# wzx99/DCFP

Hardware: AMD Instinct MI355X
Metric: training images/sec at 1024x2048 DeepLabv3-R101 (higher is better)
Workload: dtype f32; 1 GPU; DeepLabv3-resnet101+ASPP os8, 4x3x1024x2048 per GPU, CE+0.4*deepsup CE (fused upsample), 3x3 stride-1 convs with >= 256 channels as fp32 Winograd F(2x2,3x3) (fwd / dgrad / wgrad), all other convs direct implicit GEMM, EIC step, SGD m0.9 wd5e-4; global_batch=4, parallelism=dp1

## Files before the change

dcfp_amd/_lib.py:

```python
import ctypes as C
import os
import subprocess
import threading

_HERE = os.path.dirname(os.path.abspath(__file__))
LIB_PATH = os.environ.get("DCFP_LIB") or os.path.join(_HERE, "libdcfp_hip.so")
CSRC = os.path.join(_HERE, "csrc")

_lib = None
_lock = threading.Lock()


class ConvDesc(C.Structure):
    _fields_ = [(n, C.c_int32) for n in
                ("N", "Cin", "H", "W", "Cout", "KH", "KW", "stride", "pad", "dil", "Hout", "Wout",
                 "x_pitch", "dy_pitch")]


class ConvF16Desc(C.Structure):
    _fields_ = [(n, C.c_int32) for n in
                ("N", "H", "W", "Cin8", "x_pitch", "Cout", "K", "stride", "pad", "dil", "Hout", "Wout",
                 "y_pitch", "y_off", "res_pitch", "res_off", "relu")]


# ... 86 lines not shown
    "dcfp_p2p_import": (_I, [_P, C.POINTER(C.c_void_p)]),
    "dcfp_p2p_unmap": (_I, [_P]),
    "dcfp_syncbn_p2p_exchange_f32": (_I, [C.POINTER(C.c_void_p), _I, _I, C.c_uint32, _I, _P, _I, _I, _P, _R,
                                          C.c_uint32, _P, _P]),
    "dcfp_bn_apply_relu_mask_f32": (_I, [_P, _P, _P, _P, _P, _F, _P, _P, _P, _I, _I, _I, _P]),
    "dcfp_conv2d_fwd_stat_slots": (_L, [_D, _P, _L]),
    "dcfp_conv2d_fwd_stats_f32_nchw": (_I, [_D, _P, _P, _P, _L, _P, _P, _Z, _I, _P]),
    "dcfp_bn_stats_from_partials_f32": (_I, [_P, _L, _I, _I, _P, _P, _R, _P]),
    "dcfp_bn_bwd_apply_f32": (_I, [_P, _L, _P, _P, _L, _P, _P, _P, _P, _F, _P, _P, _F, _P, _I, _P, _P,
                                   _I, _I, _I, _I, _I, _P]),
    "dcfp_bn_bwd_fused_sync_bytes": (_Z, [_I, _I, _I]),
    "dcfp_bn_bwd_fused_f32": (_I, [_P, _L, _P, _P, _L, _P, _P, _P, _P, _F, _F, _I, _P, _P, _I, _I, _I, _I, _I,
                                   _P, _P, _P, _P, _P, _Z, C.c_uint32, C.c_uint32, _P, _P]),
    "dcfp_maxpool3x3s2_fwd_f32": (_I, [_P, _P, _P, _I, _I, _I, _I, _I, _I, _P]),
    "dcfp_maxpool3x3s2_bwd_f32": (_I, [_P, _P, _P, _I, _I, _I, _I, _I, _I, _P]),
    "dcfp_rowsum_f32": (_I, [_P, _L, _P, _F, _I, _I, _I, _P]),
    "dcfp_broadcast_hw_f32": (_I, [_P, _F, _P, _L, _I, _I, _I, _I, _P]),
    "dcfp_add_f32": (_I, [_P, _P, _P, _L, _P]),
    "dcfp_channel_scale_f32": (_I, [_P, _P, _P, _I, _I, _I, _P]),
    "dcfp_upsample_bilinear_fwd_f32": (_I, [_P, _P, _I, _I, _I, _I, _I, _I, _I, _P]),
    "dcfp_upsample_bilinear_bwd_f32": (_I, [_P, _P, _I, _I, _I, _I, _I, _I, _I, _P]),
    "dcfp_resize_bilinear_into_f32": (_I, [_P, _L, _I, _I, _I, _I, _P, _L, _I, _I, _I, _I, _P]),
    "dcfp_resize_bilinear_adjoint_f32": (_I, [_P, _L, _I, _I, _I, _I, _I, _P, _L, _I, _I, _I, _I, _P]),
    "dcfp_ppm_pool_f32": (_I, [_P, _I, _I, _I, _I, _I, _P, _P, _I, _P, _L, _I, _P]),
    "dcfp_ppm_pool_adjoint_f32": (_I, [_P, _I, _I, _I, _I, _I, _P, _P, _L, _I, _P, _P]),
    "dcfp_ppm_resize_adjoint_f32": (_I, [_P, _L, _I, _I, _I, _I, _I, _P, _P, _I, _P]),
    "dcfp_upsample_ce_workspace_bytes": (_Z, [_I, _I, _I]),
    "dcfp_upsample_ce_fwd_f32": (_I, [_P, _P, _P, _I, _I, _I, _I, _I, _I, _I, _I, _P, _P, _P, _P,
                                      _Z, _P]),
    "dcfp_upsample_ce_bwd_f32": (_I, [_P, _P, _P, _I, _I, _I, _I, _I, _I, _I, _I, _P, _P, _P, _P]),
# ... 74 lines not shown
```

dcfp_amd/csrc/bn.hip:

```cpp
#include "common.h"
#include <stdlib.h>

namespace {

constexpr int kThreads = 256;

__device__ __forceinline__ float bn_val(float v, float mu, float istd, float g, float b) {
    return fmaf((v - mu) * istd, g, b);
}

struct BnPlan {
    int chunks;
    int chunk_elems;
};

constexpr int kChunkElems = 8192;

BnPlan bn_plan(int N, int C, int HW) {
    const long long E = (long long)N * HW;
    long long chunks = (E + kChunkElems - 1) / kChunkElems;
    if (E <= kChunkElems) {
        const long long by_size = (E + 2047) / 2048;
        long long by_grid = 4096 / (C > 0 ? C : 1);
        if (by_grid < 1) by_grid = 1;
// ... 951 lines not shown
```

dcfp_amd/csrc/common.h:

```cpp
#pragma once
#include <hip/hip_runtime.h>
#include <stdint.h>
#include <stddef.h>
#include "../../include/dcfp_hip.h"

#define DCFP_WAVE 64

#define DCFP_RETURN_LAUNCH()                         \
    do {                                             \
        hipError_t e__ = hipGetLastError();          \
        return (e__ == hipSuccess) ? DCFP_OK : (int)e__; \
    } while (0)

struct Igemm2Red {
    const float* x;
    const unsigned long long* mask;
    const float* mean;
    float* part;
};

static inline hipStream_t dcfp_s(dcfp_stream_t s) { return reinterpret_cast<hipStream_t>(s); }

static inline bool dcfp_aligned16(const void* p) { return (reinterpret_cast<uintptr_t>(p) & 15u) == 0; }

// ... 12 lines not shown
    for (int off = 32; off > 0; off >>= 1) v += __shfl_down(v, off, 64);
    return v;
}

__device__ __forceinline__ float block_sum_256(float v, float* smem ) {
    v = wave_sum(v);
    const int lane = threadIdx.x & 63, wid = threadIdx.x >> 6;
    if (lane == 0) smem[wid] = v;
    __syncthreads();
    float r = 0.f;
    if (threadIdx.x == 0) r = (smem[0] + smem[1]) + (smem[2] + smem[3]);
    __syncthreads();
    return r;
}

__device__ __forceinline__ void running_update(const DcfpBnRunning& r, int c, float mean, float var, float n) {
    if (r.running_mean) {
#pragma clang fp contract(off)
        const float unb = n / fmaxf(n - 1.0f, 1.0f);
        const float keep = 1.0f - r.momentum;
        const float a = r.running_mean[c] * keep, b = r.momentum * mean;
        r.running_mean[c] = a + b;
        const float vu = var * unb;
        const float d = r.running_var[c] * keep, e = r.momentum * vu;
        r.running_var[c] = d + e;
    }
    if (c == 0 && r.num_batches_tracked) r.num_batches_tracked[0] += 1;
}
```

dcfp_amd/csrc/conv_igemm2.hip:

```cpp
#include "igemm2_common.h"
#include <queue>
#include <vector>
#include <stdio.h>
#include <stdlib.h>

namespace {

__device__ __forceinline__ int wp_row(int m, int perm8) {
    if (!perm8) return m;
    const int j = m & 255;
    return (m & ~255) + 32 * (j & 7) + (j >> 3);
}

__global__ void __launch_bounds__(256)
permute_weights_kernel(const float* __restrict__ w, float* __restrict__ wp, int T, int Ck, int CkP,
                       int M, int Mpad, int sAm, int sAc, int perm8) {
    const long long total = (long long)T * CkP * Mpad;
    for (long long i = (long long)blockIdx.x * 256 + threadIdx.x; i < total;
         i += (long long)gridDim.x * 256) {
        const int m = wp_row((int)(i % Mpad), perm8);
        const long long r = i / Mpad;
        const int c = (int)(r % CkP);
        const int t = (int)(r / CkP);
        float v = 0.f;
// ... 24 lines not shown
        return;
    }
    const long long total = (long long)e.T * e.CkP * e.Mpad;
#pragma unroll
    for (int u = 0; u < kWpBlockElems / 256; ++u) {
        const long long i = base + u * 256 + threadIdx.x;
        if (i >= total) return;
        const int m = wp_row((int)(i % e.Mpad), e.perm8);
        const long long r = i / e.Mpad;
        const int c = (int)(r % e.CkP);
        const int t = (int)(r / e.CkP);
        float v = 0.f;
        if (m < e.M && c < e.Ck) v = e.w[(long long)m * e.sAm + (long long)c * e.sAc + t];
        e.wp[i] = v;
    }
}

__device__ __forceinline__ float half_xor(float v, int mask) {
    switch (mask) {
        case 1: return __builtin_bit_cast(float, __builtin_amdgcn_ds_swizzle(__builtin_bit_cast(int, v), (1 << 10) | 0x1f));
        case 2: return __builtin_bit_cast(float, __builtin_amdgcn_ds_swizzle(__builtin_bit_cast(int, v), (2 << 10) | 0x1f));
        case 4: return __builtin_bit_cast(float, __builtin_amdgcn_ds_swizzle(__builtin_bit_cast(int, v), (4 << 10) | 0x1f));
        case 8: return __builtin_bit_cast(float, __builtin_amdgcn_ds_swizzle(__builtin_bit_cast(int, v), (8 << 10) | 0x1f));
        default: return __builtin_bit_cast(float, __builtin_amdgcn_ds_swizzle(__builtin_bit_cast(int, v), (16 << 10) | 0x1f));
    }
}

template <int TAPS, int TM, int TN, int WM, int WN, bool SD, bool ACC, int KB = 16>
__global__ void __launch_bounds__(64 * WM * WN, (TM * TN <= 8 && WM * WN == 4 && !ACC) ? 2 : 1)
igemm2_kernel(const Igemm2Params p) {
// ... 915 lines not shown
    if (pick_tapskip(p, 256) == 0) return 1.0;
    long long live = 0;
    for (int ti = 0; ti < p.tiles_per_img; ++ti) live += tile_live_rows(p, ti);
    return (double)live / (3.0 * p.tiles_per_img);
}

void dcfp_igemm2_wp_layout(int T, int M, int Ck, int P, long long px, int sn, int sd, int off0, int offstep, int HiWi,
                           int Wo, bool pitched, int sAm, int sAc, DcfpWpEntry* e) {
    const TileCfg c = pick_cfg(M, px, sd);
    const bool d8 = dcfp_igemm2_use_dma8(T, M, P, px, sn, sd, off0, offstep, HiWi, Wo, pitched);
    e->T = T; e->Ck = Ck; e->CkP = round_up(Ck, ck_pad()); e->M = M; e->Mpad = round_up(M, d8 ? 256 : c.bm);
    e->sAm = sAm; e->sAc = sAc; e->perm8 = d8 ? 1 : 0;
}

int dcfp_igemm2_permute_multi(const DcfpWpEntry* table, int n, long long total_blocks, hipStream_t stream) {
    hipLaunchKernelGGL(permute_weights_multi_kernel, dim3((unsigned)total_blocks), dim3(256), 0, stream, table, n);
    DCFP_RETURN_LAUNCH();
}

bool dcfp_igemm2_persist() {
    static const bool persist = [] { const char* e = getenv("DCFP_IGEMM_PERSIST"); return !e || atoi(e) != 0; }();
    return persist;
}

bool dcfp_igemm2_dma_shape(int T, int M, int Ck, int P, long long px, int sn, int sd, int off0, int HiWi, int Wo) {
    static const bool dma = [] { const char* e = getenv("DCFP_IGEMM_DMA"); return !e || atoi(e) != 0; }();
    static const bool dma9 = [] { const char* e = getenv("DCFP_IGEMM_DMA9"); return !e || atoi(e) != 0; }();
    if (!dma || pick_cfg(M, px, sd).id != 4 || sn != 1 || sd != 1 || HiWi != P || Wo % 4 != 0) return false;
    return T == 1 ? off0 == 0 : dma9;
}

// ... 106 lines not shown
```

dcfp_amd/csrc/igemm2_common.h:

```cpp
#pragma once
#include "common.h"
#include <type_traits>

struct Igemm2Params {
    const float* in;
    const float* wp;
    const float* bias;
    const float* scale;
    const float* shift;
    const float* residual;
    int relu;
    float* out;
    long long in_nstride, out_nstride;
    int N, M, Mpad, Ck, CkP;
    int Hi, Wi, Ho, Wo, P, tiles_per_img, tiles_n_total, tiles_m;
    int sn, sd, off0, offstep;
    int accumulate, vec_store;
    int tile2d;
    int Hc, Wc, tiles_per_phase;
    int in_pitch;
    int zfold;
    const float* fan_src;
    const unsigned long long* fan_mask;
    long long wp_nstride;
// ... 10 lines not shown

typedef float f32x16 __attribute__((ext_vector_type(16)));
typedef float f32x4 __attribute__((ext_vector_type(4)));

constexpr int BK = 16;
constexpr unsigned kOob = 0x80000000u;

template <int I, int N, typename F>
__device__ __forceinline__ void static_for(F&& f) {
    if constexpr (I < N) {
        f(std::integral_constant<int, I>{});
        static_for<I + 1, N>(f);
    }
}

__device__ __forceinline__ void wino_filter2_pair(const float* __restrict__ w, int sAm, int sAc, int flip, int M, int Ck,
                                                  int Mpad, long long idx, float* __restrict__ Ug) {
    const int mblocks = Mpad / 64;
    const int c = (int)(idx / Mpad), m = (int)(idx - (long long)c * Mpad);
    float g[9];
    if (m < M && c < Ck) {
        const float* src = w + (long long)m * sAm + (long long)c * sAc;
#pragma unroll
        for (int t = 0; t < 9; ++t) g[t] = src[flip ? 8 - t : t];
    } else {
#pragma unroll
        for (int t = 0; t < 9; ++t) g[t] = 0.f;
    }
    float r[4][3];
#pragma unroll
    for (int k = 0; k < 3; ++k) {
        const float g0 = g[k], g1 = g[3 + k], g2 = g[6 + k];
        r[0][k] = g0;
        r[1][k] = 0.5f * ((g0 + g2) + g1);
        r[2][k] = 0.5f * ((g0 + g2) - g1);
        r[3][k] = g2;
    }
    const int cb = c >> 3, cl = c & 7, mb = m >> 6, ml = m & 63;
    float* dst = Ug + ((((long long)(cb * mblocks + mb) * 16) * 2 + (ml >> 5)) * 64 + (cl & 1) * 32 + (ml & 31)) * 4 + (cl >> 1);
#pragma unroll
    for (int i = 0; i < 4; ++i) {
        const float a = r[i][0], b = r[i][1], cc = r[i][2];
        dst[(4 * i + 0) * 512] = a;
        dst[(4 * i + 1) * 512] = 0.5f * ((a + cc) + b);
        dst[(4 * i + 2) * 512] = 0.5f * ((a + cc) - b);
        dst[(4 * i + 3) * 512] = cc;
    }
}

template <int T>
struct Frag;
template <>
struct Frag<4> {
    static __device__ __forceinline__ void ld(const float* p, float (&f)[4]) {
        const float4 v = *reinterpret_cast<const float4*>(p);
        f[0] = v.x; f[1] = v.y; f[2] = v.z; f[3] = v.w;
    }
};
template <>
struct Frag<2> {
    static __device__ __forceinline__ void ld(const float* p, float (&f)[2]) {
        const float2 v = *reinterpret_cast<const float2*>(p);
// ... 10 lines not shown
```

dcfp_amd/csrc/pool.hip:

```cpp
#include "common.h"
#include <math.h>

namespace {

constexpr int kThreads = 256;

__global__ void __launch_bounds__(kThreads)
maxpool3x3s2_fwd_kernel(const float* __restrict__ x, float* __restrict__ y,
                        int32_t* __restrict__ argmax, long long total, int H, int W, int Hout,
                        int Wout) {
    for (long long idx = (long long)blockIdx.x * kThreads + threadIdx.x; idx < total;
         idx += (long long)gridDim.x * kThreads) {
        const int ow = (int)(idx % Wout);
        const long long t = idx / Wout;
        const int oh = (int)(t % Hout);
        const long long plane = t / Hout;
        const float* xp = x + plane * (long long)H * W;
        const int h0 = oh * 2 - 1, w0 = ow * 2 - 1;
        const int hs = h0 < 0 ? 0 : h0, ws = w0 < 0 ? 0 : w0;
        const int he = h0 + 3 > H ? H : h0 + 3, we = w0 + 3 > W ? W : w0 + 3;
        float best = -INFINITY;
        int bi = hs * W + ws;
        for (int h = hs; h < he; ++h) {
            for (int w = ws; w < we; ++w) {
// ... 21 lines not shown
    const float* xp = x + plane * (long long)H * W;
    const int h0 = 2 * oh - 1, c0 = 2 * ow0;
    float best[4] = {-INFINITY, -INFINITY, -INFINITY, -INFINITY};
    const int hs = h0 < 0 ? 0 : h0;
    int bi[4];
#pragma unroll
    for (int j = 0; j < 4; ++j) bi[j] = hs * W + ((c0 + 2 * j - 1) < 0 ? 0 : (c0 + 2 * j - 1));
#pragma unroll
    for (int r = 0; r < 3; ++r) {
        const int h = h0 + r;
        if (h < 0 || h >= H) continue;
        const float* row = xp + (long long)h * W;
        const float4 a = *reinterpret_cast<const float4*>(row + c0);
        const float4 b = *reinterpret_cast<const float4*>(row + c0 + 4);
        const float v[9] = {c0 > 0 ? row[c0 - 1] : 0.f, a.x, a.y, a.z, a.w, b.x, b.y, b.z, b.w};
#pragma unroll
        for (int j = 0; j < 4; ++j) {
#pragma unroll
            for (int k = 0; k < 3; ++k) {
                if (k == 0 && j == 0 && c0 == 0) continue;
                const float t = v[2 * j + k];
                if (t > best[j] || t != t) { best[j] = t; bi[j] = h * W + c0 + 2 * j + k - 1; }
            }
        }
    }
    const long long o = rowid * Wout + ow0;
    *reinterpret_cast<float4*>(y + o) = make_float4(best[0], best[1], best[2], best[3]);
    *reinterpret_cast<int4*>(argmax + o) = make_int4(bi[0], bi[1], bi[2], bi[3]);
}

// ... 161 lines not shown
    if (Hout != (H + 2 - 3) / 2 + 1 || Wout != (W + 2 - 3) / 2 + 1) return DCFP_E_BADDESC;
    if ((long long)H * W > 0x7fffffffLL) return DCFP_E_UNSUPPORTED;
    const long long total = (long long)N * C * Hout * Wout;
    const long long orows = (long long)N * C * Hout;
    const int segs = (Wout / 4 + kThreads - 1) / kThreads;
    if (W % 8 == 0 && dcfp_aligned16(x) && dcfp_aligned16(y) && dcfp_aligned16(argmax) &&
        orows * segs <= 0x7fffffffLL)
        hipLaunchKernelGGL(maxpool3x3s2_fwd_vec4_kernel, dim3((unsigned)(orows * segs)), dim3(kThreads), 0,
                           dcfp_s(stream), x, y, argmax, H, W, Hout, Wout, segs);
    else
        hipLaunchKernelGGL(maxpool3x3s2_fwd_kernel, dim3(stream_grid(total)), dim3(kThreads), 0,
                           dcfp_s(stream), x, y, argmax, total, H, W, Hout, Wout);
    DCFP_RETURN_LAUNCH();
}

extern "C" int dcfp_maxpool3x3s2_bwd_f32(const float* dy, const int32_t* argmax, float* dx, int N,
                                         int C, int H, int W, int Hout, int Wout,
                                         dcfp_stream_t stream) {
    if (!dy || !dx || !argmax || N <= 0 || C <= 0 || H <= 0 || W <= 0) return DCFP_E_BADDESC;
    if (Hout != (H + 2 - 3) / 2 + 1 || Wout != (W + 2 - 3) / 2 + 1) return DCFP_E_BADDESC;
    const long long total = (long long)N * C * H * W;
    const long long rows = (long long)N * C * H;
    const int segs = (W / 4 + kThreads - 1) / kThreads;
    if (W % 4 == 0 && dcfp_aligned16(dx) && rows * segs <= 0x7fffffffLL)
        hipLaunchKernelGGL(maxpool3x3s2_bwd_vec4_kernel, dim3((unsigned)(rows * segs)), dim3(kThreads), 0,
                           dcfp_s(stream), dy, argmax, dx, H, W, Hout, Wout, segs);
    else
        hipLaunchKernelGGL(maxpool3x3s2_bwd_kernel, dim3(stream_grid(total)), dim3(kThreads), 0,
                           dcfp_s(stream), dy, argmax, dx, total, H, W, Hout, Wout);
    DCFP_RETURN_LAUNCH();
// ... 44 lines not shown
```

dcfp_amd/networks/_exec.py:

```python
import os

import torch
import torch.nn as nn

from .. import ops

_BN_TYPES = (nn.BatchNorm2d, nn.SyncBatchNorm)


def conv(m, x):
    if m.groups != 1 or m.kernel_size[0] != m.kernel_size[1] or m.stride[0] != m.stride[1] \
            or m.padding[0] != m.padding[1] or m.dilation[0] != m.dilation[1] \
            or isinstance(m.padding, str) or m.padding_mode != "zeros":
        raise RuntimeError(f"dcfp_amd: unsupported conv configuration {m}")
    return ops.conv2d(x, m.weight, m.bias, m.stride[0], m.padding[0], m.dilation[0])


FUSE_BLOCKS = os.environ.get("DCFP_NO_BLOCK_FUSION") is None


def _bn_args(m):
    training = m.training or (m.running_mean is None)
    sync = False
    if isinstance(m, nn.SyncBatchNorm) and training:
# ... 43 lines not shown
            shift = bn.bias - bn.running_mean * scale
        cached = (key, scale.contiguous(), shift.contiguous())
        bn._dcfp_fold = cached
    return cached[1], cached[2]


def conv_bn_act(cm, bn, x, relu=False, residual=None, next_conv=None):
    if (not bn.training) and bn.running_mean is not None and not torch.is_grad_enabled() \
            and cm.bias is None and cm.groups == 1 and cm.padding_mode == "zeros":
        scale, shift = _fold(bn)
        return ops.conv2d_fused_infer(x, cm.weight, scale, shift, cm.stride[0], cm.padding[0],
                                      cm.dilation[0], residual, relu)
    return bn_act(bn, conv(cm, x), relu=relu, residual=residual, prev_conv=cm, next_conv=next_conv)


def _plain_conv(m, k):
    ok = (m.groups == 1 and m.bias is None and m.kernel_size == (k, k) and m.padding_mode == "zeros"
          and not isinstance(m.padding, str))
    if not ok:
        raise RuntimeError(f"dcfp_amd: unsupported conv configuration in Bottleneck: {m}")


def bottleneck(blk, x):
    _plain_conv(blk.conv1, 1); _plain_conv(blk.conv2, 3); _plain_conv(blk.conv3, 1)
    bns = [blk.bn1, blk.bn2, blk.bn3]
    tensors = [blk.conv1.weight, blk.bn1.weight, blk.bn1.bias, blk.conv2.weight, blk.bn2.weight,
               blk.bn2.bias, blk.conv3.weight, blk.bn3.weight, blk.bn3.bias]
    stride, dil = blk.conv2.stride[0], blk.conv2.dilation[0]
    if blk.conv2.padding[0] != dil or blk.conv1.stride[0] != 1 or blk.conv3.stride[0] != 1:
        raise RuntimeError("dcfp_amd: unexpected Bottleneck geometry")
# ... 54 lines not shown
```

dcfp_amd/networks/backbone/resnet.py:

```python
import torch.nn as nn

from .. import _exec
from ... import ops

BatchNorm2d = nn.BatchNorm2d

_DEPTHS = {"50": [3, 4, 6, 3], "101": [3, 4, 23, 3], "152": [3, 8, 36, 3]}
_OS_CFG = {16: ([1, 2, 2, 1], [1, 1, 1, 2]), 8: ([1, 2, 1, 1], [1, 1, 2, 4]),
           32: ([1, 2, 2, 2], [1, 1, 1, 1])}


class Bottleneck(nn.Module):
    expansion = 4

    def __init__(self, inplanes, planes, stride=1, dilation=1, downsample=None):
        super().__init__()
        self.conv1 = nn.Conv2d(inplanes, planes, kernel_size=1, bias=False)
        self.bn1 = BatchNorm2d(planes)
        self.conv2 = nn.Conv2d(planes, planes, kernel_size=3, stride=stride, dilation=dilation,
                               padding=dilation, bias=False)
        self.bn2 = BatchNorm2d(planes)
        self.conv3 = nn.Conv2d(planes, planes * 4, kernel_size=1, bias=False)
        self.bn3 = BatchNorm2d(planes * 4)
        self.relu = nn.ReLU(inplace=True)
# ... 37 lines not shown
        if stride != 1 or self.inplanes != planes * block.expansion:
            downsample = nn.Sequential(
                nn.Conv2d(self.inplanes, planes * block.expansion, kernel_size=1, stride=stride,
                          bias=False),
                BatchNorm2d(planes * block.expansion))
        blocks = [block(self.inplanes, planes, stride, block_dilations[0], downsample)]
        self.inplanes = planes * block.expansion
        for d in block_dilations[1:]:
            blocks.append(block(self.inplanes, planes, dilation=d))
        return nn.Sequential(*blocks)

    def forward(self, input):
        _exec.require_device(input)
        stem = list(self.conv1.children())
        x = _exec.run_sequential(nn.Sequential(*stem[:-1]), input, tail_conv=stem[-1])
        x = _exec.conv_bn_act(stem[-1], self.bn1, x, relu=True)
        x = ops.maxpool3x3s2(x)
        outs = []
        for i in range(1, 5):
            for blk in getattr(self, "layer" + str(i)):
                x = blk(x)
            if i in self.out_index:
                if i < 4:
                    tap, x = ops.fork(x)
                    outs.append(tap)
                else:
                    outs.append(x)
        return tuple(outs)


def build_resnet(name, para):
    para = para if para is not None else {}
# ... 17 lines not shown
```

dcfp_amd/ops.py:

```python
import ctypes as C
import os
import weakref

import torch
import torch.distributed as dist

from . import _lib, arena, syncbn_p2p
from ._lib import ConvDesc, BnRunning, check

_ws_cache = {}
WEIGHT_EPOCH = [0]

_PROFILE = None


def profile_start():
    global _PROFILE
    _PROFILE = []


def profile_stop():
    global _PROFILE
    recs, _PROFILE = _PROFILE, None
    torch.cuda.synchronize()
# ... 134 lines not shown


def _desc(xshape, wshape, stride, pad, dil, x_pitch=0, dy_pitch=0):
    N, Cin, H, W = xshape
    Cout, Cin2, KH, KW = wshape
    if Cin2 != Cin:
        raise RuntimeError(f"conv2d: weight expects {Cin2} input channels, got {Cin} (groups unsupported)")
    d = ConvDesc(N, Cin, H, W, Cout, KH, KW, stride, pad, dil,
                 conv_out_size(H, KH, stride, pad, dil), conv_out_size(W, KW, stride, pad, dil),
                 x_pitch, dy_pitch)
    return d


FUSE_BN_STATS = os.environ.get("DCFP_FUSED_BN_STATS", "1") not in ("0",)
BN_RELU_BITMASK = os.environ.get("DCFP_BN_RELU_BITMASK", "1") not in ("0",)
SYNCBN_ASYNC = os.environ.get("DCFP_SYNCBN_ASYNC", "1") not in ("0",)


_WP_OWNERS = weakref.WeakSet()
_WP_TABLE = {"version": 0, "built": -1, "dev": None, "n": 0, "blocks": 0, "entries": []}


def _wp_buffer(w, which, d, nbytes, variant=""):
    key = (which, d.N, d.H, d.W, d.stride, d.pad, d.dil, d.x_pitch, d.dy_pitch, variant)
    tag = (w.data_ptr(), w._version, WEIGHT_EPOCH[0], torch.cuda.current_stream().cuda_stream)
    cache = getattr(w, "_dcfp_wp", None)
    if cache is None:
        cache = {}
        try:
            w._dcfp_wp = cache
# ... 322 lines not shown
        st = y.stride()
        ypitch = _pitch_of(y)
        if not ypitch and st[3] == 1 and st[2] > W and st[2] % 4 == 0 and st[1] == H * st[2]:
            ypitch = st[2]
        if tuple(y.shape) != tuple(x.shape) or (not ypitch and (st[3] != 1 or st[2] != W or st[1] != H * W)):
            raise RuntimeError("bn_apply: out must have dense images or be a row-pitched buffer")
        yns = st[0]
    nbytes = (8.0 + (4.0 if residual is not None else 0.0)) * x.numel()
    _timed("bn_apply", None, nbytes, lambda: check(
        _lib.lib().dcfp_bn_apply_f32(_p(x), _p(mean), _p(var), _p(gamma), _p(beta), float(eps),
                                     _p(residual), int(relu), _p(y), yns, N, Cc, H * W, W, ypitch, _stream()),
        "bn_apply"))
    return y


def bn_apply_relu_mask(x, mean, var, gamma, beta, eps, residual):
    N, Cc, H, W = x.shape
    if (H * W) % 256 != 0:
        return None
    x = x.contiguous(); residual = residual.contiguous()
    y = torch.empty_like(x)
    mask = torch.empty(x.numel() // 64, dtype=torch.int64, device=x.device)
    rc = [0]

    def run():
        rc[0] = _lib.lib().dcfp_bn_apply_relu_mask_f32(_p(x), _p(mean), _p(var), _p(gamma), _p(beta), float(eps),
                                                       _p(residual), _p(y), _p(mask), N, Cc, H * W, _stream())
    _timed("bn_apply", None, 12.125 * x.numel(), run)
    if rc[0] == _lib.E_UNSUPPORTED:
        return None
# ... 187 lines not shown
            work = px.exchange_async(both, out, 1)
            return out[:Cc], out[Cc:], work
        _timed("syncbn_p2p_bwd", None, 8.0 * Cc * px.world, lambda: px.exchange(both, out, 1))
        return out[:Cc], out[Cc:]
    if adjacent:
        both = s1.as_strided((2 * Cc,), (1,), s1.storage_offset())
        work = dist.all_reduce(both, group=group, async_op=async_op)
        return (s1, s2, work) if async_op else (s1, s2)
    both = torch.cat([s1, s2])
    work = dist.all_reduce(both, group=group, async_op=async_op)
    r1, r2 = both[:Cc], both[Cc:]
    return (r1, r2, work) if async_op else (r1.contiguous(), r2.contiguous())


def bn_forward_impl(x, gamma, beta, running_mean, running_var, residual, relu, training,
                    momentum, eps, sync, nbt=None, stats=None, want_mask=False, out=None):
    _require(x, "x")
    x = x.contiguous()
    N, Cc, H, W = x.shape
    count = float(N * H * W)
    group = _sync_group(sync) if training else None
    if training:
        run = _bn_run(running_mean, running_var, momentum, nbt)
        if stats is not None:
            mean, var, applied = stats
            if applied:
                run = None
        elif group is None:
            mean, var = bn_stats(x, run)
            run = None
        else:
# ... 1 lines not shown
        if group is not None:
            mean, var, count = sync_bn_stats(mean, var, count, group, run)
        elif run is not None:
            if running_mean is not None and momentum is not None:
                check(_lib.lib().dcfp_bn_update_running_f32(
                    _p(mean), _p(var), Cc, float(momentum), float(count), None, _p(running_mean),
                    _p(running_var), _stream()), "bn_update_running")
            if nbt is not None:
                nbt.add_(1)
    else:
        mean, var = running_mean, running_var
    if want_mask and relu and residual is not None and BN_RELU_BITMASK and out is None:
        ym = bn_apply_relu_mask(x, mean, var, gamma, beta, eps, residual)
        if ym is not None:
            return ym[0], (mean, var, count, group, ym[1])
    y = bn_apply(x, mean, var, gamma, beta, eps, residual, relu, out=out)
    return y, (mean, var, count, group)


def _bn_bwd_preface(relu, y, state, gamma, beta, gparam, bparam):
    mask = state[4] if len(state) > 4 else None
    if relu and mask is not None:
        relu, y = 3, mask
    else:
        relu = (1 if y is not None else 2) if relu else 0
    gp = gparam if gparam is not None else gamma
    bp = bparam if bparam is not None else beta
    return (relu, y, gp) + tuple(arena.grad_target(gp)) + (bp,) + tuple(arena.grad_target(bp))


# ... 112 lines not shown
        ctx.cfg = (relu, training, eps, residual is not None)
        return y

    @staticmethod
    def backward(ctx, dy):
        x, y = ctx.saved_tensors[:2]
        gamma, beta = ctx.params
        relu, training, eps, has_res = ctx.cfg
        state = _bn_state(ctx.meta, ctx.saved_tensors[2:], 0)
        need_res = has_res and ctx.needs_input_grad[5]
        dx_out = pitched_buffer(tuple(x.shape), ctx.dx_pitch, ctx.dx_key, x.device) if ctx.dx_pitch else None
        dx, dgamma, dbeta, dres = bn_backward_impl(dy, x, y, gamma, beta, state, relu, training, eps, need_res,
                                                   dx_out=dx_out)
        _release_pitch(ctx)
        return dx, dgamma, dbeta, None, None, dres, None, None, None, None, None, None, None


class BottleneckFn(torch.autograd.Function):

    @staticmethod
    def forward(ctx, x, cfg, *tensors):
        ctx.prev_rec = getattr(x, "_dcfp_bn3_rec", None) if FANIN_BN_SUMS else None
        x = x.contiguous()
        has_ds = len(tensors) == 12
        w1, g1, b1, w2, g2, b2, w3, g3, b3 = tensors[:9]
        bnargs = cfg["bn"]
        stride, dil = cfg["stride"], cfg["dil"]

        N_, _, H_, W_ = x.shape
        y1_shape = (N_, w1.shape[0], H_, W_)
# ... 955 lines not shown
```

include/dcfp_hip.h:

```cpp
#ifndef DCFP_HIP_H
#define DCFP_HIP_H

#include <stddef.h>
#include <stdint.h>

#ifdef __cplusplus
extern "C" {
#endif

#define DCFP_OK 0
#define DCFP_E_BADDESC (-1)
#define DCFP_E_UNSUPPORTED (-2)
#define DCFP_E_WORKSPACE (-3)

typedef void* dcfp_stream_t;

int dcfp_abi_version(void);

typedef struct DcfpConvDesc {
    int32_t N, Cin, H, W;
    int32_t Cout, KH, KW;
    int32_t stride, pad, dil;
    int32_t Hout, Wout;
    int32_t x_pitch, dy_pitch;
// ... 121 lines not shown

size_t dcfp_bn_bwd_fused_sync_bytes(int N, int C, int HW);
int dcfp_bn_bwd_fused_f32(const float* dy, int64_t dy_nstride, const float* x, const float* y,
                          int64_t y_nstride, const float* mean, const float* var, const float* gamma,
                          const float* beta, float eps, float count, int relu, float* dx, float* d_residual,
                          int N, int C, int HW, int W, int dx_pitch, float* sum_dy, float* sum_dy_xmu,
                          float* dgamma, float* dbeta, void* sync, size_t sync_bytes, uint32_t epoch,
                          uint32_t spin_limit, int32_t* status, dcfp_stream_t stream);

int dcfp_maxpool3x3s2_fwd_f32(const float* x, float* y, int32_t* argmax,
                              int N, int C, int H, int W, int Hout, int Wout,
                              dcfp_stream_t stream);
int dcfp_maxpool3x3s2_bwd_f32(const float* dy, const int32_t* argmax, float* dx,
                              int N, int C, int H, int W, int Hout, int Wout,
                              dcfp_stream_t stream);
int dcfp_rowsum_f32(const float* x, int64_t x_nstride, float* y, float scale,
                    int N, int C, int HW, dcfp_stream_t stream);
int dcfp_broadcast_hw_f32(const float* v, float scale, float* y, int64_t y_nstride,
                          int accumulate, int N, int C, int HW, dcfp_stream_t stream);
int dcfp_add_f32(const float* a, const float* b, float* out, int64_t n,
                 dcfp_stream_t stream);
int dcfp_channel_scale_f32(const float* x, const float* mask, float* y,
                           int N, int C, int HW, dcfp_stream_t stream);

int dcfp_upsample_bilinear_fwd_f32(const float* x, float* y, int N, int C,
                                   int h, int w, int H, int W, int align_corners,
                                   dcfp_stream_t stream);
int dcfp_upsample_bilinear_bwd_f32(const float* dy, float* dx, int N, int C,
                                   int h, int w, int H, int W, int align_corners,
                                   dcfp_stream_t stream);
// ... 182 lines not shown
```

Baseline: 12.26 images/s.

## Fuse stem BN+ReLU into maxpool and tile weight permutation through LDS

The stem's BN apply and ReLU now run inside the 3x3 stride-2 max-pool kernel, so the full-resolution activated tensor is never written and read back. A new autograd function saves the pre-BN input and argmax and recomputes through maxpool backward followed by BN backward. Separately, the weight-permutation kernel gets a transposed, LDS-tiled variant, including a tiled Winograd filter-transform path, so reads and writes are coalesced. The extra dz buffer in backward and the differences in the BN backward path are the main risks.

```diff
diff --git a/dcfp_amd/_lib.py b/dcfp_amd/_lib.py
--- a/dcfp_amd/_lib.py
+++ b/dcfp_amd/_lib.py
@@ -124,6 +124,7 @@
                                    _P, _P, _P, _P, _P, _Z, C.c_uint32, C.c_uint32, _P, _P]),
     "dcfp_maxpool3x3s2_fwd_f32": (_I, [_P, _P, _P, _I, _I, _I, _I, _I, _I, _P]),
     "dcfp_maxpool3x3s2_bwd_f32": (_I, [_P, _P, _P, _I, _I, _I, _I, _I, _I, _P]),
+    "dcfp_bn_relu_maxpool3x3s2_fwd_f32": (_I, [_P, _P, _P, _P, _P, _F, _P, _P, _I, _I, _I, _I, _I, _I, _P]),
     "dcfp_rowsum_f32": (_I, [_P, _L, _P, _F, _I, _I, _I, _P]),
     "dcfp_broadcast_hw_f32": (_I, [_P, _F, _P, _L, _I, _I, _I, _I, _P]),
     "dcfp_add_f32": (_I, [_P, _P, _P, _L, _P]),
diff --git a/dcfp_amd/csrc/bn.hip b/dcfp_amd/csrc/bn.hip
--- a/dcfp_amd/csrc/bn.hip
+++ b/dcfp_amd/csrc/bn.hip
@@ -5,9 +5,6 @@
 
 constexpr int kThreads = 256;
 
-__device__ __forceinline__ float bn_val(float v, float mu, float istd, float g, float b) {
-    return fmaf((v - mu) * istd, g, b);
-}
 
 struct BnPlan {
     int chunks;
diff --git a/dcfp_amd/csrc/common.h b/dcfp_amd/csrc/common.h
--- a/dcfp_amd/csrc/common.h
+++ b/dcfp_amd/csrc/common.h
@@ -50,6 +50,10 @@
     return r;
 }
 
+__device__ __forceinline__ float bn_val(float v, float mu, float istd, float g, float b) {
+    return fmaf((v - mu) * istd, g, b);
+}
+
 __device__ __forceinline__ void running_update(const DcfpBnRunning& r, int c, float mean, float var, float n) {
     if (r.running_mean) {
 #pragma clang fp contract(off)
diff --git a/dcfp_amd/csrc/conv_igemm2.hip b/dcfp_amd/csrc/conv_igemm2.hip
--- a/dcfp_amd/csrc/conv_igemm2.hip
+++ b/dcfp_amd/csrc/conv_igemm2.hip
@@ -62,6 +62,158 @@
         if (m < e.M && c < e.Ck) v = e.w[(long long)m * e.sAm + (long long)c * e.sAc + t];
         e.wp[i] = v;
     }
+}
+
+constexpr int kWpRows = kWpBlockElems / 32;
+__device__ __forceinline__ void permute_tile(const float* __restrict__ w, float* __restrict__ wp, int T, int Ck, int CkP,
+                                             int M, int Mpad, int sAm, int sAc, int perm8, long long blk,
+                                             float* __restrict__ tile ) {
+    const int R = T * CkP;
+    const long long rows_total = (long long)R * (Mpad >> 5);
+    const long long g0 = blk * kWpRows;
+    const int tid = threadIdx.x;
+    if (sAc <= sAm) {
+        const int pl = tid & 63;
+        const long long g = g0 + pl;
+        if (g < rows_total) {
+            const int strip = (int)(g / R), p = (int)(g - (long long)strip * R);
+            const int c = p / T, t = p - c * T;
+#pragma unroll
+            for (int u = 0; u < 8; ++u) {
+                const int ml = 4 * u + (tid >> 6);
+                const int m = wp_row(32 * strip + ml, perm8);
+                float v = 0.f;
+                if (m < M && c < Ck) v = w[(long long)m * sAm + (long long)c * sAc + t];
+                tile[pl * 33 + ml] = v;
+            }
+        }
+    } else {
+        const int ml = tid & 31;
+#pragma unroll
+        for (int u = 0; u < 8; ++u) {
+            const int pl = 8 * u + (tid >> 5);
+            const long long g = g0 + pl;
+            if (g >= rows_total) break;
+            const int strip = (int)(g / R), p = (int)(g - (long long)strip * R);
+            const int c = p / T, t = p - c * T;
+            const int m = wp_row(32 * strip + ml, perm8);
+            float v = 0.f;
+            if (m < M && c < Ck) v = w[(long long)m * sAm + (long long)c * sAc + t];
+            tile[pl * 33 + ml] = v;
+        }
+    }
+    __syncthreads();
+    {
+        const int ml = tid & 31;
+#pragma unroll
+        for (int u = 0; u < 8; ++u) {
+            const int pl = 8 * u + (tid >> 5);
+            const long long g = g0 + pl;
+            if (g >= rows_total) break;
+            const int strip = (int)(g / R), p = (int)(g - (long long)strip * R);
+            const int c = p / T, t = p - c * T;
+            wp[((long long)t * CkP + c) * Mpad + 32 * strip + ml] = tile[pl * 33 + ml];
+        }
+    }
+}
+
+constexpr int kWinoFwdPitch = 73, kWinoDgPitch = 581;
+constexpr int kWinoTileLds = 64 * kWinoFwdPitch;
+__device__ __forceinline__ void wino_filter2_tiles(const DcfpWpEntry& e, long long blk, float* __restrict__ lds) {
+    const bool fwd = e.sAc == 9;
+    const int flip = e.perm8 == 3;
+    const int mblocks = e.Mpad / 64;
+    const long long ntiles = (long long)(e.CkP / 8) * mblocks;
+    const int tid = threadIdx.x;
+#pragma unroll 1
+    for (int j = 0; j < 4; ++j) {
+        const long long tile = blk * 4 + j;
+        if (tile >= ntiles) break;
+        const int cb = (int)(tile / mblocks), mb = (int)(tile - (long long)cb * mblocks);
+        if (fwd) {
+            const int cols = min(72, (e.Ck - 8 * cb) * 9);
+#pragma unroll 2
+            for (int f = tid; f < 64 * 72; f += 256) {
+                const int row = f / 72, col = f - row * 72, m = 64 * mb + row;
+                float v = 0.f;
+                if (m < e.M && col < cols) v = e.w[(long long)m * e.sAm + (long long)cb * 72 + col];
+                lds[row * kWinoFwdPitch + col] = v;
+            }
+        } else {
+            const int cols = min(576, (e.M - 64 * mb) * 9);
+#pragma unroll 2
+            for (int f = tid; f < 8 * 576; f += 256) {
+                const int row = f / 576, col = f - row * 576, c = 8 * cb + row;
+                float v = 0.f;
+                if (c < e.Ck && col < cols) v = e.w[(long long)c * e.sAc + (long long)mb * 576 + col];
+                lds[row * kWinoDgPitch + col] = v;
+            }
+        }
+        __syncthreads();
+        float* out = e.wp + tile * (16 * 512);
+#pragma unroll
+        for (int h = 0; h < 2; ++h) {
+            const int o = h * 256 + tid;
+            const int lane = (o >> 2) & 63;
+            const int cl = 2 * (o & 3) + (lane >> 5), ml = 32 * (o >> 8) + (lane & 31);
+            const float* src = fwd ? lds + ml * kWinoFwdPitch + cl * 9 : lds + cl * kWinoDgPitch + ml * 9;
+            float g[9];
+#pragma unroll
+            for (int t = 0; t < 9; ++t) g[t] = src[flip ? 8 - t : t];
+            wino_filter2_store(g, out + o);
+        }
+        __syncthreads();
+    }
+}
+
+__global__ void __launch_bounds__(256)
+permute_weights_multi_t_kernel(const DcfpWpEntry* __restrict__ table, int n) {
+    __shared__ float tile[kWinoTileLds];
+    static_assert(kWinoTileLds >= 8 * kWinoDgPitch && kWinoTileLds >= kWpRows * 33, "one LDS array for all three paths");
+    const long long blk = blockIdx.x;
+    int lo = 0, hi = n - 1;
+    while (lo < hi) {
+        const int mid = (lo + hi + 1) >> 1;
+        if (table[mid].first_block <= blk) lo = mid; else hi = mid - 1;
+    }
+    const DcfpWpEntry e = table[lo];
+    if (e.perm8 >= 2 && (e.sAc == 9 || e.sAm == 9) && e.CkP % 8 == 0 && e.Mpad % 64 == 0) {
+        wino_filter2_tiles(e, blk - e.first_block, tile);
+        return;
+    }
+    if (e.perm8 >= 2) {
+        const long long base = (blk - e.first_block) * kWpBlockElems;
+        const long long pairs = (long long)e.CkP * e.Mpad;
+#pragma unroll 1
+        for (int u = 0; u < kWpBlockElems / 256; ++u) {
+            const long long i = base + u * 256 + threadIdx.x;
+            if (i >= pairs) return;
+            wino_filter2_pair(e.w, e.sAm, e.sAc, e.perm8 == 3, e.M, e.Ck, e.Mpad, i, e.wp);
+        }
+        return;
+    }
+    if (e.Mpad & 31) {
+        const long long base = (blk - e.first_block) * kWpBlockElems;
+        const long long total = (long long)e.T * e.CkP * e.Mpad;
+        for (int u = 0; u < kWpBlockElems / 256; ++u) {
+            const long long i = base + u * 256 + threadIdx.x;
+            if (i >= total) return;
+            const int m = wp_row((int)(i % e.Mpad), e.perm8);
+            const long long r = i / e.Mpad;
+            const int c = (int)(r % e.CkP);
+            const int t = (int)(r / e.CkP);
+            float v = 0.f;
+            if (m < e.M && c < e.Ck) v = e.w[(long long)m * e.sAm + (long long)c * e.sAc + t];
+            e.wp[i] = v;
+        }
+        return;
+    }
+    permute_tile(e.w, e.wp, e.T, e.Ck, e.CkP, e.M, e.Mpad, e.sAm, e.sAc, e.perm8, blk - e.first_block, tile);
+}
+
+bool wp_transpose() {
+    static const bool on = [] { const char* e = getenv("DCFP_WP_TRANSPOSE"); return !e || atoi(e) != 0; }();
+    return on;
 }
 
 __device__ __forceinline__ float half_xor(float v, int mask) {
@@ -1007,7 +1159,10 @@
 }
 
 int dcfp_igemm2_permute_multi(const DcfpWpEntry* table, int n, long long total_blocks, hipStream_t stream) {
-    hipLaunchKernelGGL(permute_weights_multi_kernel, dim3((unsigned)total_blocks), dim3(256), 0, stream, table, n);
+    if (wp_transpose())
+        hipLaunchKernelGGL(permute_weights_multi_t_kernel, dim3((unsigned)total_blocks), dim3(256), 0, stream, table, n);
+    else
+        hipLaunchKernelGGL(permute_weights_multi_kernel, dim3((unsigned)total_blocks), dim3(256), 0, stream, table, n);
     DCFP_RETURN_LAUNCH();
 }
 
diff --git a/dcfp_amd/csrc/igemm2_common.h b/dcfp_amd/csrc/igemm2_common.h
--- a/dcfp_amd/csrc/igemm2_common.h
+++ b/dcfp_amd/csrc/igemm2_common.h
@@ -48,6 +48,26 @@
     }
 }
 
+__device__ __forceinline__ void wino_filter2_store(const float (&g)[9], float* __restrict__ dst) {
+    float r[4][3];
+#pragma unroll
+    for (int k = 0; k < 3; ++k) {
+        const float g0 = g[k], g1 = g[3 + k], g2 = g[6 + k];
+        r[0][k] = g0;
+        r[1][k] = 0.5f * ((g0 + g2) + g1);
+        r[2][k] = 0.5f * ((g0 + g2) - g1);
+        r[3][k] = g2;
+    }
+#pragma unroll
+    for (int i = 0; i < 4; ++i) {
+        const float a = r[i][0], b = r[i][1], cc = r[i][2];
+        dst[(4 * i + 0) * 512] = a;
+        dst[(4 * i + 1) * 512] = 0.5f * ((a + cc) + b);
+        dst[(4 * i + 2) * 512] = 0.5f * ((a + cc) - b);
+        dst[(4 * i + 3) * 512] = cc;
+    }
+}
+
 __device__ __forceinline__ void wino_filter2_pair(const float* __restrict__ w, int sAm, int sAc, int flip, int M, int Ck,
                                                   int Mpad, long long idx, float* __restrict__ Ug) {
     const int mblocks = Mpad / 64;
@@ -61,25 +81,9 @@
 #pragma unroll
         for (int t = 0; t < 9; ++t) g[t] = 0.f;
     }
-    float r[4][3];
-#pragma unroll
-    for (int k = 0; k < 3; ++k) {
-        const float g0 = g[k], g1 = g[3 + k], g2 = g[6 + k];
-        r[0][k] = g0;
-        r[1][k] = 0.5f * ((g0 + g2) + g1);
-        r[2][k] = 0.5f * ((g0 + g2) - g1);
-        r[3][k] = g2;
-    }
     const int cb = c >> 3, cl = c & 7, mb = m >> 6, ml = m & 63;
     float* dst = Ug + ((((long long)(cb * mblocks + mb) * 16) * 2 + (ml >> 5)) * 64 + (cl & 1) * 32 + (ml & 31)) * 4 + (cl >> 1);
-#pragma unroll
-    for (int i = 0; i < 4; ++i) {
-        const float a = r[i][0], b = r[i][1], cc = r[i][2];
-        dst[(4 * i + 0) * 512] = a;
-        dst[(4 * i + 1) * 512] = 0.5f * ((a + cc) + b);
-        dst[(4 * i + 2) * 512] = 0.5f * ((a + cc) - b);
-        dst[(4 * i + 3) * 512] = cc;
-    }
+    wino_filter2_store(g, dst);
 }
 
 template <int T>
diff --git a/dcfp_amd/csrc/pool.hip b/dcfp_amd/csrc/pool.hip
--- a/dcfp_amd/csrc/pool.hip
+++ b/dcfp_amd/csrc/pool.hip
@@ -59,6 +59,92 @@
         const float4 a = *reinterpret_cast<const float4*>(row + c0);
         const float4 b = *reinterpret_cast<const float4*>(row + c0 + 4);
         const float v[9] = {c0 > 0 ? row[c0 - 1] : 0.f, a.x, a.y, a.z, a.w, b.x, b.y, b.z, b.w};
+#pragma unroll
+        for (int j = 0; j < 4; ++j) {
+#pragma unroll
+            for (int k = 0; k < 3; ++k) {
+                if (k == 0 && j == 0 && c0 == 0) continue;
+                const float t = v[2 * j + k];
+                if (t > best[j] || t != t) { best[j] = t; bi[j] = h * W + c0 + 2 * j + k - 1; }
+            }
+        }
+    }
+    const long long o = rowid * Wout + ow0;
+    *reinterpret_cast<float4*>(y + o) = make_float4(best[0], best[1], best[2], best[3]);
+    *reinterpret_cast<int4*>(argmax + o) = make_int4(bi[0], bi[1], bi[2], bi[3]);
+}
+
+__device__ __forceinline__ float bn_relu_val(float v, float mu, float istd, float g, float b) {
+    const float o = bn_val(v, mu, istd, g, b);
+    return o > 0.f ? o : 0.f;
+}
+
+__global__ void __launch_bounds__(kThreads)
+bn_relu_maxpool3x3s2_kernel(const float* __restrict__ x, const float* __restrict__ mean,
+                            const float* __restrict__ var, const float* __restrict__ gamma,
+                            const float* __restrict__ beta, float eps, float* __restrict__ y,
+                            int32_t* __restrict__ argmax, long long total, int C, int H, int W, int Hout, int Wout) {
+    for (long long idx = (long long)blockIdx.x * kThreads + threadIdx.x; idx < total;
+         idx += (long long)gridDim.x * kThreads) {
+        const int ow = (int)(idx % Wout);
+        const long long t = idx / Wout;
+        const int oh = (int)(t % Hout);
+        const long long plane = t / Hout;
+        const int c = (int)(plane % C);
+        const float istd = 1.0f / sqrtf(var[c] + eps);
+        const float mu = mean[c], g = gamma[c], b = beta[c];
+        const float* xp = x + plane * (long long)H * W;
+        const int h0 = oh * 2 - 1, w0 = ow * 2 - 1;
+        const int hs = h0 < 0 ? 0 : h0, ws = w0 < 0 ? 0 : w0;
+        const int he = h0 + 3 > H ? H : h0 + 3, we = w0 + 3 > W ? W : w0 + 3;
+        float best = -INFINITY;
+        int bi = hs * W + ws;
+        for (int h = hs; h < he; ++h) {
+            for (int w = ws; w < we; ++w) {
+                const float v = bn_relu_val(xp[h * W + w], mu, istd, g, b);
+                if (v > best || v != v) {
+                    best = v;
+                    bi = h * W + w;
+                }
+            }
+        }
+        y[idx] = best;
+        argmax[idx] = bi;
+    }
+}
+
+__global__ void __launch_bounds__(kThreads)
+bn_relu_maxpool3x3s2_vec4_kernel(const float* __restrict__ x, const float* __restrict__ mean,
+                                 const float* __restrict__ var, const float* __restrict__ gamma,
+                                 const float* __restrict__ beta, float eps, float* __restrict__ y,
+                                 int32_t* __restrict__ argmax, int C, int H, int W, int Hout, int Wout, int segs) {
+    const long long rowid = blockIdx.x / segs;
+    const int seg = blockIdx.x - (int)(rowid * segs);
+    const long long plane = rowid / Hout;
+    const int oh = (int)(rowid - plane * Hout);
+    const int ow0 = 4 * (seg * kThreads + threadIdx.x);
+    if (ow0 >= Wout) return;
+    const int c = (int)(plane % C);
+    const float istd = 1.0f / sqrtf(var[c] + eps);
+    const float mu = mean[c], g = gamma[c], b = beta[c];
+    const float* xp = x + plane * (long long)H * W;
+    const int h0 = 2 * oh - 1, c0 = 2 * ow0;
+    float best[4] = {-INFINITY, -INFINITY, -INFINITY, -INFINITY};
+    const int hs = h0 < 0 ? 0 : h0;
+    int bi[4];
+#pragma unroll
+    for (int j = 0; j < 4; ++j) bi[j] = hs * W + ((c0 + 2 * j - 1) < 0 ? 0 : (c0 + 2 * j - 1));
+#pragma unroll
+    for (int r = 0; r < 3; ++r) {
+        const int h = h0 + r;
+        if (h < 0 || h >= H) continue;
+        const float* row = xp + (long long)h * W;
+        const float4 p = *reinterpret_cast<const float4*>(row + c0);
+        const float4 q = *reinterpret_cast<const float4*>(row + c0 + 4);
+        const float raw[9] = {c0 > 0 ? row[c0 - 1] : 0.f, p.x, p.y, p.z, p.w, q.x, q.y, q.z, q.w};
+        float v[9];
+#pragma unroll
+        for (int k = 0; k < 9; ++k) v[k] = bn_relu_val(raw[k], mu, istd, g, b);
 #pragma unroll
         for (int j = 0; j < 4; ++j) {
 #pragma unroll
@@ -250,6 +336,27 @@
     DCFP_RETURN_LAUNCH();
 }
 
+extern "C" int dcfp_bn_relu_maxpool3x3s2_fwd_f32(const float* x, const float* mean, const float* var,
+                                                 const float* gamma, const float* beta, float eps, float* y,
+                                                 int32_t* argmax, int N, int C, int H, int W, int Hout, int Wout,
+                                                 dcfp_stream_t stream) {
+    if (!x || !mean || !var || !gamma || !beta || !y || !argmax || N <= 0 || C <= 0 || H <= 0 || W <= 0)
+        return DCFP_E_BADDESC;
+    if (Hout != (H + 2 - 3) / 2 + 1 || Wout != (W + 2 - 3) / 2 + 1) return DCFP_E_BADDESC;
+    if ((long long)H * W > 0x7fffffffLL) return DCFP_E_UNSUPPORTED;
+    const long long total = (long long)N * C * Hout * Wout;
+    const long long orows = (long long)N * C * Hout;
+    const int segs = (Wout / 4 + kThreads - 1) / kThreads;
+    if (W % 8 == 0 && dcfp_aligned16(x) && dcfp_aligned16(y) && dcfp_aligned16(argmax) &&
+        orows * segs <= 0x7fffffffLL)
+        hipLaunchKernelGGL(bn_relu_maxpool3x3s2_vec4_kernel, dim3((unsigned)(orows * segs)), dim3(kThreads), 0,
+                           dcfp_s(stream), x, mean, var, gamma, beta, eps, y, argmax, C, H, W, Hout, Wout, segs);
+    else
+        hipLaunchKernelGGL(bn_relu_maxpool3x3s2_kernel, dim3(stream_grid(total)), dim3(kThreads), 0,
+                           dcfp_s(stream), x, mean, var, gamma, beta, eps, y, argmax, total, C, H, W, Hout, Wout);
+    DCFP_RETURN_LAUNCH();
+}
+
 extern "C" int dcfp_maxpool3x3s2_bwd_f32(const float* dy, const int32_t* argmax, float* dx, int N,
                                          int C, int H, int W, int Hout, int Wout,
                                          dcfp_stream_t stream) {
diff --git a/dcfp_amd/networks/_exec.py b/dcfp_amd/networks/_exec.py
--- a/dcfp_amd/networks/_exec.py
+++ b/dcfp_amd/networks/_exec.py
@@ -81,6 +81,19 @@
     return bn_act(bn, conv(cm, x), relu=relu, residual=residual, prev_conv=cm, next_conv=next_conv)
 
 
+def conv_bn_relu_maxpool(cm, bn, x):
+    if not (ops.STEM_POOL_FUSED and bn.training and not isinstance(bn, nn.SyncBatchNorm) and x.is_cuda):
+        return ops.maxpool3x3s2(conv_bn_act(cm, bn, x, relu=True))
+    z = conv(cm, x)
+    rm, rv, training, momentum, eps, sync, nbt = _bn_args(bn)
+    pitch_cfg = None
+    if torch.is_grad_enabled() and z.requires_grad and cm.kernel_size == (3, 3):
+        dx_pitch = _conv_pitch(cm, (z.shape[0], cm.in_channels, z.shape[2], z.shape[3]))
+        if dx_pitch:
+            pitch_cfg = (bn, dx_pitch)
+    return ops.batch_norm_relu_maxpool(z, bn.weight, bn.bias, rm, rv, training, momentum, eps, sync, nbt, pitch_cfg)
+
+
 def _plain_conv(m, k):
     ok = (m.groups == 1 and m.bias is None and m.kernel_size == (k, k) and m.padding_mode == "zeros"
           and not isinstance(m.padding, str))
diff --git a/dcfp_amd/networks/backbone/resnet.py b/dcfp_amd/networks/backbone/resnet.py
--- a/dcfp_amd/networks/backbone/resnet.py
+++ b/dcfp_amd/networks/backbone/resnet.py
@@ -75,8 +75,7 @@
         _exec.require_device(input)
         stem = list(self.conv1.children())
         x = _exec.run_sequential(nn.Sequential(*stem[:-1]), input, tail_conv=stem[-1])
-        x = _exec.conv_bn_act(stem[-1], self.bn1, x, relu=True)
-        x = ops.maxpool3x3s2(x)
+        x = _exec.conv_bn_relu_maxpool(stem[-1], self.bn1, x)
         outs = []
         for i in range(1, 5):
             for blk in getattr(self, "layer" + str(i)):
diff --git a/dcfp_amd/ops.py b/dcfp_amd/ops.py
--- a/dcfp_amd/ops.py
+++ b/dcfp_amd/ops.py
@@ -172,6 +172,7 @@
 
 FUSE_BN_STATS = os.environ.get("DCFP_FUSED_BN_STATS", "1") not in ("0",)
 BN_RELU_BITMASK = os.environ.get("DCFP_BN_RELU_BITMASK", "1") not in ("0",)
+STEM_POOL_FUSED = os.environ.get("DCFP_STEM_POOL_FUSED", "1") not in ("0",)
 SYNCBN_ASYNC = os.environ.get("DCFP_SYNCBN_ASYNC", "1") not in ("0",)
 
 
@@ -524,6 +525,18 @@
     return y
 
 
+def bn_relu_maxpool(x, mean, var, gamma, beta, eps):
+    N, Cc, H, W = x.shape
+    x = x.contiguous()
+    Ho, Wo = (H + 2 - 3) // 2 + 1, (W + 2 - 3) // 2 + 1
+    y = torch.empty((N, Cc, Ho, Wo), dtype=torch.float32, device=x.device)
+    idx = torch.empty((N, Cc, Ho, Wo), dtype=torch.int32, device=x.device)
+    _timed("bn_apply", None, 4.0 * x.numel() + 8.0 * y.numel(), lambda: check(
+        _lib.lib().dcfp_bn_relu_maxpool3x3s2_fwd_f32(_p(x), _p(mean), _p(var), _p(gamma), _p(beta), float(eps), _p(y),
+                                                     _p(idx), N, Cc, H, W, Ho, Wo, _stream()), "bn_relu_maxpool"))
+    return y, idx
+
+
 def bn_apply_relu_mask(x, mean, var, gamma, beta, eps, residual):
     N, Cc, H, W = x.shape
     if (H * W) % 256 != 0:
@@ -741,7 +754,7 @@
 
 
 def bn_forward_impl(x, gamma, beta, running_mean, running_var, residual, relu, training,
-                    momentum, eps, sync, nbt=None, stats=None, want_mask=False, out=None):
+                    momentum, eps, sync, nbt=None, stats=None, want_mask=False, out=None, pool=False):
     _require(x, "x")
     x = x.contiguous()
     N, Cc, H, W = x.shape
@@ -773,6 +786,10 @@
         ym = bn_apply_relu_mask(x, mean, var, gamma, beta, eps, residual)
         if ym is not None:
             return ym[0], (mean, var, count, group, ym[1])
+    if pool:
+        if not relu or residual is not None or out is not None:
+            raise RuntimeError("bn_forward_impl: the fused max-pool tail takes BN + ReLU without residual")
+        return bn_relu_maxpool(x, mean, var, gamma, beta, eps), (mean, var, count, group)
     y = bn_apply(x, mean, var, gamma, beta, eps, residual, relu, out=out)
     return y, (mean, var, count, group)
 
@@ -915,6 +932,46 @@
                                                    dx_out=dx_out)
         _release_pitch(ctx)
         return dx, dgamma, dbeta, None, None, dres, None, None, None, None, None, None, None
+
+
+class BatchNormReluMaxPoolFn(torch.autograd.Function):
+
+    @staticmethod
+    def forward(ctx, x, gamma, beta, running_mean, running_var, training, momentum, eps, sync, nbt, pitch_cfg):
+        x = x.contiguous()
+        ctx.dx_pitch, ctx.dx_key = 0, "bn_dx"
+        if pitch_cfg is not None:
+            ctx.dx_pitch = pitch_cfg[1]
+            ctx.dx_key = ("bn_dx", id(pitch_cfg[0]))
+        (y, idx), state = bn_forward_impl(x, gamma, beta, running_mean, running_var, None, True, training, momentum,
+                                          eps, sync, nbt=nbt, pool=True)
+        flat, ctx.meta = _pack_bn_states([state])
+        ctx.save_for_backward(x, idx, *flat)
+        ctx.params = (gamma, beta)
+        ctx.cfg = (training, eps)
+        return y
+
+    @staticmethod
+    def backward(ctx, dy):
+        x, idx = ctx.saved_tensors[:2]
+        gamma, beta = ctx.params
+        training, eps = ctx.cfg
+        state = _bn_state(ctx.meta, ctx.saved_tensors[2:], 0)
+        N, Cc, H, W = x.shape
+        dy = dy.contiguous()
+        dz = torch.empty((N, Cc, H, W), dtype=torch.float32, device=dy.device)
+        check(_lib.lib().dcfp_maxpool3x3s2_bwd_f32(_p(dy), _p(idx), _p(dz), N, Cc, H, W, idx.shape[2], idx.shape[3],
+                                                   _stream()), "maxpool_bwd")
+        dx_out = pitched_buffer(tuple(x.shape), ctx.dx_pitch, ctx.dx_key, x.device) if ctx.dx_pitch else None
+        dx, dgamma, dbeta, _ = bn_backward_impl(dz, x, None, gamma, beta, state, True, training, eps, False,
+                                                dx_out=dx_out)
+        return dx, dgamma, dbeta, None, None, None, None, None, None, None, None
+
+
+def batch_norm_relu_maxpool(x, gamma, beta, running_mean, running_var, training=True, momentum=0.1, eps=1e-5,
+                            sync=False, nbt=None, pitch_cfg=None):
+    return BatchNormReluMaxPoolFn.apply(x, gamma, beta, running_mean, running_var, training, momentum, eps, sync, nbt,
+                                        pitch_cfg)
 
 
 class BottleneckFn(torch.autograd.Function):
diff --git a/include/dcfp_hip.h b/include/dcfp_hip.h
--- a/include/dcfp_hip.h
+++ b/include/dcfp_hip.h
@@ -159,6 +159,10 @@
 int dcfp_maxpool3x3s2_bwd_f32(const float* dy, const int32_t* argmax, float* dx,
                               int N, int C, int H, int W, int Hout, int Wout,
                               dcfp_stream_t stream);
+int dcfp_bn_relu_maxpool3x3s2_fwd_f32(const float* x, const float* mean, const float* var,
+                                      const float* gamma, const float* beta, float eps, float* y,
+                                      int32_t* argmax, int N, int C, int H, int W, int Hout, int Wout,
+                                      dcfp_stream_t stream);
 int dcfp_rowsum_f32(const float* x, int64_t x_nstride, float* y, float scale,
                     int N, int C, int HW, dcfp_stream_t stream);
 int dcfp_broadcast_hw_f32(const float* v, float scale, float* y, int64_t y_nstride,
```

After: 12.30 images/s (median of 6 runs). About the same (+0.3%).
